# JonasGeiping/breaching

Measured on AMD Instinct MI355X. Metric: attack iters/sec, ResNet-18 ImageNet invertinggradients; PSNR vs ref, higher is better.
Workload: dtype f32

## Files before the change

### breaching_amd/_lib.py

```python

import ctypes
import os
from ctypes import POINTER, Structure, c_char_p, c_double, c_float, c_int, c_int32, c_int64, c_uint32, c_void_p

from . import build as _build

BH_ABI_VERSION = 8
BH_GM_CHUNK = 4096
BH_GM_MAX_PTRS = 448
BH_GM_PARTIAL_STRIDE = 4
BH_GM_MAX_ROWS = 2048
BH_GM_DEFAULT_ROWS = 512
BH_GM_STAT_WORDS = 12
BH_PRIOR_MAX_GRID = 1024
BH_BN_MAX_LAYERS = 448
BH_MT_MAX_PTRS = 112
BH_BN_TILE = 4096
BH_PRIOR_PARTIAL_STRIDE = 2
BH_STATE_WORDS = 16
BH_SCHED_STRIDE = 4
GM_CACHE_AUTO, GM_CACHE_KEEP, GM_CACHE_STREAM, GM_CACHE_STREAM_ALL = 0, 1, 2, 3

GM_KINDS = {
    "cosine-similarity": 0,
# ... 85 lines not shown
    ),
    "bh_bn_plan_size": (
        c_int,
        [c_int32, POINTER(c_int32), POINTER(c_int32), POINTER(c_int32), POINTER(c_int64), POINTER(c_int64), POINTER(c_int64),
         POINTER(c_int64), POINTER(c_int64)],
    ),
    "bh_bn_plan_build": (
        c_int,
        [c_int32, POINTER(c_int32), POINTER(c_int32), POINTER(c_int32), POINTER(c_float), POINTER(BnLayer), POINTER(BnItem),
         c_int64, POINTER(BnItem), c_int64],
    ),
    "bh_bn_bwd_accumulate": (c_int, [c_void_p, c_void_p, c_int32, c_void_p, c_void_p, c_int64, c_void_p, c_void_p, c_void_p, c_void_p]),
    "bh_bn_eval_fwd": (c_int, [c_void_p] * 8 + [c_int32, c_int32, c_int32, c_int32, c_void_p]),
    "bh_bn_eval_slabs": (c_int32, [c_int32, c_int32, c_int32]),
    "bh_bn_eval_bwd": (c_int, [c_void_p] * 14 + [c_int32, c_int32, c_int32, c_void_p]),
    "bh_bn_eval_bwd_bwd": (c_int, [c_void_p] * 14 + [c_int32, c_int32, c_int32, c_void_p]),
    "bh_bn_eval_bwd_bwd2": (c_int, [c_void_p] * 15 + [c_int32, c_int32, c_int32, c_void_p]),
    "bh_ln_fwd": (c_int, [c_void_p] * 6 + [c_int32, c_int32, ctypes.c_float, c_void_p]),
    "bh_ln_bwd": (c_int, [c_void_p] * 8 + [c_int32, c_int32, c_void_p]),
    "bh_ln_bwd_bwd": (c_int, [c_void_p] * 12 + [c_int32, c_int32, c_void_p]),
    "bh_bn_sums": (c_int, [c_int32, POINTER(c_void_p), POINTER(c_int32), c_void_p, c_void_p, c_int64, c_void_p, c_int32, c_int32, c_void_p]),
    "bh_bn_finalize": (c_int, [c_int32, c_void_p, c_void_p, c_void_p, c_void_p, c_void_p, c_void_p, c_void_p, c_void_p, c_int32, c_void_p]),
    "bh_bn_bwd": (
        c_int,
        [c_int32, POINTER(c_void_p), POINTER(c_int32), c_void_p, c_void_p, c_int64, c_void_p, c_void_p, c_void_p, c_void_p],
    ),
    "bh_mt_num_groups": (c_int32, [c_int32]),
    "bh_mt_group_bounds": (c_int, [c_int32, POINTER(GmChunk), c_int64, POINTER(c_int32)]),
    "bh_mt_axpy": (
        c_int,
# ... 87 lines not shown
```

### breaching_amd/attacker.py

```python

import copy
import logging
import time
from collections import defaultdict

import numpy as np
import torch

from . import _lib, schedules, streams as trial_streams, trials, workers
from .config import cfg_get as _cfg_get
from .gm import objective_lookup
from .priors import HipNormRegularization, HipTotalVariation, launch_tv_norm, regularizer_lookup
from .victim_layers import (FusedEpilogueError, _ConvFunction, _ConvGradFunction, _EvalAffineBatchNorm2d, _EvalBNFunction,
                            _EvalBNGradFunction, _HipConv2d, _HipLayerNorm, owned_conv_grad_enabled, use_owned_conv_gradient,
                            _launch_eval_bn, _LayerNormFunction, _LayerNormGradFunction, _PendingBatchNorm, _under_functorch,
                            fast_eval_bn_enabled, fast_eval_bn_mode, fast_layer_norm_enabled, fuse_bn_relu_enabled, fuse_bn_relu_policy,
                            use_affine_eval_batchnorm, use_hip_layernorm)

log = logging.getLogger(__name__)

embedding_layer_names = ["encoder.weight", "word_embeddings.weight", "transformer.wte"]

_DEFAULT_SETUP = dict(dtype=torch.float, device=torch.device("cpu"))


class HipOptimizationAttacker:

    def __init__(self, model, loss_fn, cfg_attack, setup=_DEFAULT_SETUP):
        self.cfg = cfg_attack
        self.memory_format = torch.channels_last if cfg_attack.impl.mixed_precision else torch.contiguous_format
        self.setup = dict(device=torch.device(setup["device"]), dtype=getattr(torch, cfg_attack.impl.dtype))
# ... 122 lines not shown
            optimal = self._select_optimal_reconstruction(local_solutions, local_scores, stats, shard)
            timing["select_s"] = time.perf_counter() - t_select
            if pool is not None:
                pool.timing["select_s"] = round(timing["select_s"], 4)
                pool.finish()
        except BaseException:
            if pool is not None:
                pool.abort()
                if pool.closed:
                    self._pool = None
            raise
        timing["total_s"] = time.perf_counter() - t_call
        stats["execution"] = dict(trials=stats.pop("execution_trials"), pool=pool.describe() if pool is not None else None,
                                  fused_epilogue_fallback=getattr(self, "fused_epilogue_fallback", None),
                                  owned_conv_grad=owned_conv_grad_enabled(self.cfg),
                                  pool_fallback=getattr(self, "_pool_fallback", None), world=shard.world,
                                  trial_streams=trial_streams.calibration_report(self.setup["device"]),
                                  timing={k: round(v, 4) for k, v in timing.items()})
        reconstructed_data = self._package(optimal, labels)
        if server_payload[0]["metadata"].modality == "text":
            raw = reconstructed_data["data"]
            reconstructed_data = self._postprocess_text_data(reconstructed_data)
            self._attach_raw_embeddings(reconstructed_data, raw)
        if "ClassAttack" in server_secrets:
            true_num_data = server_secrets["ClassAttack"]["true_num_data"]
            full = torch.zeros([true_num_data, *self.data_shape], **self.setup)
            full[server_secrets["ClassAttack"]["target_indx"]] = optimal if torch.is_tensor(optimal) else optimal[0]
            reconstructed_data["data"] = full
            reconstructed_data["labels"] = server_secrets["ClassAttack"]["all_labels"]
        return reconstructed_data, stats
# ... 107 lines not shown
                new_model.train()
                for module in new_model.modules():
                    if hasattr(module, "track_running_stats"):
                        module.reset_parameters()
                        module.track_running_stats = False
                buffers = []
            with torch.no_grad():
                for param, server_state in zip(new_model.parameters(), payload["parameters"]):
                    param.copy_(server_state.to(**self.setup))
                for buffer, server_state in zip(new_model.buffers(), buffers):
                    buffer.copy_(server_state.to(**self.setup))
            if self.cfg.impl.JIT is not None:
                raise NotImplementedError("impl.JIT (torch.jit script/trace of the victim model) is not supported.")
            bn_mode = fast_eval_bn_mode(self.cfg)
            if bn_mode is not None:
                use_affine_eval_batchnorm(new_model, bn_mode, fuse_epilogue=fuse_bn_relu_enabled(self.cfg))
            if fast_layer_norm_enabled(self.cfg):
                use_hip_layernorm(new_model)
            if owned_conv_grad_enabled(self.cfg):
                use_owned_conv_gradient(new_model)
            models.append(new_model)
        return models

    def _cast_shared_data(self, shared_data):
        for data in shared_data:
            data["gradients"] = [g.to(**self.setup) for g in data["gradients"]]
            if data["buffers"] is not None:
                data["buffers"] = [b.to(device=self.setup["device"], dtype=self.setup["dtype"]) for b in data["buffers"]]
        return shared_data

    def _normalize_gradients(self, shared_data, fudge_factor=1e-6):
        for data in shared_data:
            grad_norm = torch.stack([g.pow(2).sum() for g in data["gradients"]]).sum().sqrt()
            torch._foreach_div_(data["gradients"], max(grad_norm, fudge_factor))
        return shared_data
# ... 839 lines not shown
```

### breaching_amd/csrc/affine_kernels.hip

```cpp

#include "bh_common.h"

namespace {

using bh::kBlock;


struct ChannelWalk {
  int c, slab, lane, lanes;
  bool active;
};

__device__ __forceinline__ ChannelWalk channel_of(int C, int S, bool narrow) {
  ChannelWalk w;
  if (narrow) {
    w.c = blockIdx.x * bh::kWavesPerBlock + (threadIdx.x >> 6);
    w.slab = 0;
    w.lane = threadIdx.x & (bh::kWave - 1);
    w.lanes = bh::kWave;
  } else {
    w.c = blockIdx.x / S;
    w.slab = blockIdx.x - w.c * S;
    w.lane = threadIdx.x;
    w.lanes = kBlock;
// ... 103 lines not shown
        flush();
      }
    }
    sums[0] += (double)a0;
    sums[1] += (double)a1;
  }
  if (stats == nullptr) return;
  channel_sum<2>(sums, narrow != 0, lds);
  if (w.active && w.lane == 0) {
    double* out = stats + 2 * ((size_t)w.c * S + w.slab);
    out[0] = sums[0];
    out[1] = sums[1];
  }
}

__global__ __launch_bounds__(kBlock) void bn_eval_bwd_kernel(const float* __restrict__ gy, const float* __restrict__ x,
                                                             const float* __restrict__ weight, const float* __restrict__ inv_std,
                                                             const float* __restrict__ mean_inv, float* __restrict__ gx,
                                                             float* __restrict__ gw, float* __restrict__ gb,
                                                             double* __restrict__ part, const float* __restrict__ tap_coef,
                                                             const float* __restrict__ tap_gout, const float* __restrict__ ymask,
                                                             float* __restrict__ gres, const float* __restrict__ add_in, int B, int C,
                                                             int HW, int S, int narrow) {
  __shared__ double lds[bh::kWavesPerBlock * 2];
  const ChannelWalk w = channel_of(C, S, narrow != 0);
  double v[2] = {0.0, 0.0};
  if (w.active) {
    const float s = (weight ? weight[w.c] : 1.f) * inv_std[w.c];
    float ta = 0.f, tb = 0.f;
    if (tap_coef) {
      const float2 ab = reinterpret_cast<const float2*>(tap_coef)[w.c];
      const float g0 = tap_gout ? tap_gout[0] : 1.f;
      ta = g0 * ab.x;
      tb = g0 * ab.y;
    }
    const bool vec = (HW & 3) == 0;
    uint32_t unit, v0, v1;
    slab_range(B, HW, S, w.slab, vec, unit, v0, v1);
    const size_t cstride = (size_t)C * unit, cbase = (size_t)w.c * unit;
    float a0 = 0.f, a1 = 0.f;
    int cnt = 0;
    auto flush = [&]() {
      if (cnt >= 32) {
        v[0] += (double)a0;
        v[1] += (double)a1;
        a0 = a1 = 0.f;
        cnt = 0;
      }
    };
    if (vec) {
      const float4* __restrict__ gy4 = reinterpret_cast<const float4*>(gy);
      const float4* __restrict__ x4 = reinterpret_cast<const float4*>(x);
      const float4* m4 = reinterpret_cast<const float4*>(ymask ? ymask : gy);
      const float4* __restrict__ e4 = reinterpret_cast<const float4*>(add_in);
      float4* __restrict__ gres4 = reinterpret_cast<float4*>(gres);
      float4* __restrict__ gx4 = reinterpret_cast<float4*>(gx);
      const float4 zero = make_float4(0.f, 0.f, 0.f, 0.f);
      const uint32_t step = (uint32_t)w.lanes;
      for (uint32_t u0 = v0 + (uint32_t)w.lane; u0 < v1; u0 += step * kStage) {
        float4 gv[kStage], qv[kStage], mv[kStage], ev[kStage];
        size_t at[kStage];
#pragma unroll
        for (int k = 0; k < kStage; ++k) {
          const uint32_t u = u0 + (uint32_t)k * step;
          at[k] = slab_offset(u < v1 ? u : u0, B, unit, cstride, cbase);
          gv[k] = gy4[at[k]];
          qv[k] = x4[at[k]];
          mv[k] = m4[at[k]];
          ev[k] = zero;
          if (gx && add_in) ev[k] = e4[at[k]];
        }
#pragma unroll
        for (int k = 0; k < kStage; ++k) {
          const uint32_t u = u0 + (uint32_t)k * step;
          if (u < v1) {
            float4 g = gv[k];
            const float4 q = qv[k];
            if (ymask) {
              const float4 m = mv[k];
              g = make_float4(m.x <= 0.f ? 0.f : g.x, m.y <= 0.f ? 0.f : g.y, m.z <= 0.f ? 0.f : g.z, m.w <= 0.f ? 0.f : g.w);
            }
            if (gres) gres4[at[k]] = g;
            if (gx) {
              float4 o = make_float4(g.x * s, g.y * s, g.z * s, g.w * s);
              if (tap_coef) o = make_float4(o.x + fmaf(tb, q.x, ta), o.y + fmaf(tb, q.y, ta), o.z + fmaf(tb, q.z, ta), o.w + fmaf(tb, q.w, ta));
              if (add_in) {
                const float4 e = ev[k];
                o = make_float4(o.x + e.x, o.y + e.y, o.z + e.z, o.w + e.w);
              }
              gx4[at[k]] = o;
            }
            a0 += (g.x + g.y) + (g.z + g.w);
            a1 = fmaf(g.x, q.x, a1);
            a1 = fmaf(g.y, q.y, a1);
            a1 = fmaf(g.z, q.z, a1);
            a1 = fmaf(g.w, q.w, a1);
            cnt += 4;
            flush();
          }
        }
      }
    } else {
      for (uint32_t u = v0 + (uint32_t)w.lane; u < v1; u += (uint32_t)w.lanes) {
        const size_t at = slab_offset(u, B, unit, cstride, cbase);
        float g = gy[at];
        const float q = x[at];
        if (ymask && ymask[at] <= 0.f) g = 0.f;
        if (gres) gres[at] = g;
        if (gx) gx[at] = (tap_coef ? g * s + fmaf(tb, q, ta) : g * s) + (add_in ? add_in[at] : 0.f);
        a0 += g;
        a1 = fmaf(g, q, a1);
        cnt += 1;
        flush();
      }
    }
    v[0] += (double)a0;
    v[1] += (double)a1;
  }
  channel_sum<2>(v, narrow != 0, lds);
  if (w.active && w.lane == 0) {
    if (S > 1) {
      part[((size_t)w.c * S + w.slab) * 2] = v[0];
      part[((size_t)w.c * S + w.slab) * 2 + 1] = v[1];
// ... 159 lines not shown

int bh_bn_eval_fwd(const float* x, const float* weight, const float* bias, const float* inv_std, const float* mean_inv, float* y,
                   double* stats, const float* residual, int32_t relu, int32_t B, int32_t C, int32_t HW, void* stream) {
  if (!eval_bn_args_ok(x, inv_std, mean_inv, B, C, HW) || y == nullptr) return BH_EINVAL;
  if ((reinterpret_cast<uintptr_t>(stats) & 7u) != 0 || (relu != 0 && relu != 1)) return BH_EINVAL;
  if ((HW & 3) == 0 &&
      ((reinterpret_cast<uintptr_t>(x) | reinterpret_cast<uintptr_t>(y) | reinterpret_cast<uintptr_t>(residual)) & 15u) != 0)
    return BH_EINVAL;
  int S = 1, narrow = 0;
  const int grid = eval_bn_grid(B, C, HW, S, narrow);
  hipLaunchKernelGGL(bn_eval_fwd_kernel, dim3(grid), dim3(kBlock), 0, bh::as_stream(stream), x, weight, bias, inv_std, mean_inv,
                     y, stats, residual, relu, B, C, HW, S, narrow);
  return bh::launch_status();
}

int bh_bn_eval_bwd(const float* gy, const float* x, const float* weight, const float* inv_std, const float* mean_inv, float* gx,
                   float* gw, float* gb, double* workspace, const float* tap_coef, const float* tap_gout, const float* y_mask,
                   float* g_residual, const float* gx_add, int32_t B, int32_t C, int32_t HW, void* stream) {
  if (!eval_bn_args_ok(x, inv_std, mean_inv, B, C, HW) || gy == nullptr) return BH_EINVAL;
  if ((reinterpret_cast<uintptr_t>(tap_coef) & 7u) != 0 || ((tap_coef != nullptr || gx_add != nullptr) && gx == nullptr)) return BH_EINVAL;
  if ((HW & 3) == 0 && ((reinterpret_cast<uintptr_t>(x) | reinterpret_cast<uintptr_t>(gy) | reinterpret_cast<uintptr_t>(gx) |
                         reinterpret_cast<uintptr_t>(y_mask) | reinterpret_cast<uintptr_t>(g_residual) | reinterpret_cast<uintptr_t>(gx_add)) & 15u) != 0)
    return BH_EINVAL;
  int S = 1, narrow = 0;
  const int grid = eval_bn_grid(B, C, HW, S, narrow);
  if (S > 1 && workspace == nullptr) return BH_EINVAL;
  hipStream_t st = bh::as_stream(stream);
  hipLaunchKernelGGL(bn_eval_bwd_kernel, dim3(grid), dim3(kBlock), 0, st, gy, x, weight, inv_std, mean_inv, gx, gw, gb, workspace,
                     tap_coef, tap_gout, y_mask, g_residual, gx_add, B, C, HW, S, narrow);
  if (S > 1 && (gw != nullptr || gb != nullptr))
    hipLaunchKernelGGL(bn_eval_combine_kernel<2>, dim3((C + kBlock - 1) / kBlock), dim3(kBlock), 0, st, workspace, inv_std,
                       mean_inv, gw, gb, C, S);
  return bh::launch_status();
}

int bh_bn_eval_bwd_bwd2(const float* ggx, const float* ggx2, const float* ggw, const float* ggb, const float* gy, const float* x,
                        const float* weight, const float* inv_std, const float* mean_inv, float* d_gy, float* d_x, float* d_w,
                        double* workspace, const float* y_mask, const float* gg_residual, int32_t B, int32_t C, int32_t HW, void* stream) {
  if (!eval_bn_args_ok(x, inv_std, mean_inv, B, C, HW) || gy == nullptr) return BH_EINVAL;
  if (ggx2 != nullptr && ggx == nullptr) return BH_EINVAL;
  if ((HW & 3) == 0 && ((reinterpret_cast<uintptr_t>(x) | reinterpret_cast<uintptr_t>(gy) | reinterpret_cast<uintptr_t>(ggx) |
                         reinterpret_cast<uintptr_t>(ggx2) | reinterpret_cast<uintptr_t>(d_gy) | reinterpret_cast<uintptr_t>(d_x) | reinterpret_cast<uintptr_t>(y_mask) |
                         reinterpret_cast<uintptr_t>(gg_residual)) & 15u) != 0)
    return BH_EINVAL;
  int S = 1, narrow = 0;
  const int grid = eval_bn_grid(B, C, HW, S, narrow);
  if (S > 1 && workspace == nullptr) return BH_EINVAL;
  hipStream_t st = bh::as_stream(stream);
// ... 17 lines not shown
```

### breaching_amd/victim_layers.py

```python

import torch

from . import _lib
from .config import cfg_get as _cfg_get

def _vector_ready(t, hw):
    if not t.is_contiguous():
        t = t.contiguous()
    if hw % 4 == 0 and t.data_ptr() % 16:
        t = t.clone()
    return t


def _under_functorch(x):
    try:
        from torch._C._functorch import is_functorch_wrapped_tensor, peek_interpreter_stack

        return bool(is_functorch_wrapped_tensor(x)) or peek_interpreter_stack() is not None
    except Exception:
        return False


class _EvalBNFunction(torch.autograd.Function):

    @staticmethod
    def forward(ctx, x, weight, bias, inv_std, mean_inv, stats=None, tap=None, residual=None, relu=False):
        lib = _lib.load()
        B, C = x.shape[0], x.shape[1]
        hw = x[0, 0].numel()
        xk = _vector_ready(x.detach(), hw)
        rk = None if residual is None else _vector_ready(residual.detach().to(torch.float32), hw)
        y = torch.empty_like(xk)
        with torch.cuda.device(x.device):
            _lib.check(lib.bh_bn_eval_fwd(_lib.ptr(xk), _lib.ptr(weight), _lib.ptr(bias), _lib.ptr(inv_std), _lib.ptr(mean_inv),
                                          _lib.ptr(y), _lib.ptr(stats), _lib.ptr(rk), int(bool(relu)), B, C, hw,
                                          _lib.current_stream_handle(x.device)), "bh_bn_eval_fwd")
        xp = x.view_as(x)
        ctx.save_for_backward(xp, weight, inv_std, mean_inv, *([y] if relu else []))
        ctx.has_bias, ctx.relu, ctx.has_residual = bias is not None, bool(relu), residual is not None
        ctx.tap = None if tap is None else (tap.record, tap.layer)
        ctx.set_materialize_grads(False)
        return (y, xp) if tap is None else (y, xp, x.new_empty(()))

    @staticmethod
    def backward(ctx, gy, g_xp=None, g_token=None):
        xp, weight, inv_std, mean_inv, *rest = ctx.saved_tensors
        mask = rest[0].detach() if ctx.relu else None
        none = (None,) * 9
        if g_token is None or ctx.tap is None:
            if gy is None:
                return (g_xp,) + none[1:]
            tap = None
        else:
            if torch.is_grad_enabled():
                raise NotImplementedError("The DeepInversion term fused into the BatchNorm backward supports no create_graph "
                                          "pass through it (set BREACH_HIP_BN_FUSED_TAP=0).")
            record, layer = ctx.tap
            _, coef_ptr = record.layer_coefficients(layer)
            if gy is None:
                gy = torch.zeros_like(xp)
            tap = (coef_ptr, g_token.detach().reshape(1).to(torch.float32), record.coef)
        fold = g_xp is not None and not torch.is_grad_enabled()
        gx, gw, gb, gr = _EvalBNGradFunction.apply(gy, xp, weight, inv_std, mean_inv, mask, tap, ctx.has_residual, g_xp if fold else None)
        if g_xp is not None and not fold:
            gx = gx + g_xp
        return gx, (gw if weight is not None else None), (gb if ctx.has_bias else None), None, None, None, None, gr, None


class _EvalBNGradFunction(torch.autograd.Function):

    @staticmethod
    def forward(ctx, gy, x, weight, inv_std, mean_inv, mask=None, tap=None, want_residual=False, gx_add=None):
        lib = _lib.load()
        B, C = x.shape[0], x.shape[1]
        hw = x[0, 0].numel()
        gyk = _vector_ready(gy.detach().to(torch.float32), hw)
        xk = _vector_ready(x.detach(), hw)
        mk = None if mask is None else _vector_ready(mask.detach(), hw)
        ak = None if gx_add is None else _vector_ready(gx_add.detach().to(torch.float32), hw)
        gx = torch.empty_like(xk)
        gr = torch.empty_like(xk) if want_residual else None
        gw = torch.empty(C, dtype=torch.float32, device=x.device)
        gb = torch.empty(C, dtype=torch.float32, device=x.device)
        slabs = lib.bh_bn_eval_slabs(B, C, hw)
        ws = torch.empty(2 * C * slabs, dtype=torch.float64, device=x.device) if slabs > 1 else None
        coef_ptr, gout = (tap[0], _lib.ptr(tap[1])) if tap is not None else (_lib.ptr(None), _lib.ptr(None))
        with torch.cuda.device(x.device):
            _lib.check(lib.bh_bn_eval_bwd(_lib.ptr(gyk), _lib.ptr(xk), _lib.ptr(weight), _lib.ptr(inv_std), _lib.ptr(mean_inv),
                                          _lib.ptr(gx), _lib.ptr(gw), _lib.ptr(gb), _lib.ptr(ws), coef_ptr, gout, _lib.ptr(mk), _lib.ptr(gr),
                                          _lib.ptr(ak), B, C, hw, _lib.current_stream_handle(x.device)), "bh_bn_eval_bwd")
        ctx.save_for_backward(gyk, xk, weight, inv_std, mean_inv, *([mk] if mk is not None else []))
        ctx.set_materialize_grads(False)
        ctx.extra_terms, ctx.masked = (tap is not None or gx_add is not None), mk is not None
        return gx, gw, gb, gr

    @staticmethod
    @torch.autograd.function.once_differentiable
    def backward(ctx, ggx, ggw, ggb, ggr):
        lib = _lib.load()
        gy, x, weight, inv_std, mean_inv, *rest = ctx.saved_tensors
        mask = rest[0] if ctx.masked else None
        none = (None,) * 9
        ggx2 = _take_conv_term(ctx)
        if ggx is None:
            ggx, ggx2 = ggx2, None
        if ggx is None and ggw is None and ggb is None and ggr is None:
            return none
        if ctx.extra_terms:
            raise NotImplementedError("No derivative of the BatchNorm backward with the DeepInversion term / another gradient folded in.")
        B, C = x.shape[0], x.shape[1]
        hw = x[0, 0].numel()
        ggx = None if ggx is None else _vector_ready(ggx.to(torch.float32), hw)
        ggx2 = None if ggx2 is None else _vector_ready(ggx2.to(torch.float32), hw)
        ggr = None if ggr is None else _vector_ready(ggr.to(torch.float32), hw)
        ggw = None if ggw is None else ggw.to(torch.float32).contiguous()
        ggb = None if ggb is None else ggb.to(torch.float32).contiguous()
        d_gy = torch.empty_like(x) if ctx.needs_input_grad[0] else None
        d_x = torch.empty_like(x) if (ctx.needs_input_grad[1] and ggw is not None) else None
        d_w = torch.empty(C, dtype=torch.float32, device=x.device) if (weight is not None and ctx.needs_input_grad[2] and ggx is not None) else None
        if d_gy is None and d_x is None and d_w is None:
            return none
        slabs = lib.bh_bn_eval_slabs(B, C, hw)
        ws = torch.empty(C * slabs, dtype=torch.float64, device=x.device) if slabs > 1 else None
        with torch.cuda.device(x.device):
            _lib.check(lib.bh_bn_eval_bwd_bwd2(_lib.ptr(ggx), _lib.ptr(ggx2), _lib.ptr(ggw), _lib.ptr(ggb), _lib.ptr(gy), _lib.ptr(x),
                                               _lib.ptr(weight), _lib.ptr(inv_std), _lib.ptr(mean_inv), _lib.ptr(d_gy), _lib.ptr(d_x),
                                               _lib.ptr(d_w), _lib.ptr(ws), _lib.ptr(mask), _lib.ptr(ggr), B, C, hw,
                                               _lib.current_stream_handle(x.device)), "bh_bn_eval_bwd_bwd2")
        return d_gy, d_x, d_w, None, None, None, None, None, None


def _take_conv_term(node):
    entry = getattr(node, "_conv_term", None)
    if entry is None:
        return None
    node._conv_term = None
    return entry[1] if entry[0] == torch._C._current_graph_task_id() else None


def _engine_wants(edge):
    node = edge[0] if edge is not None else None
    if node is None:
        return False
    try:
        return bool(torch._C._will_engine_execute_node(node))
    except RuntimeError:
        return True


_aten = torch.ops.aten


class _ConvFunction(torch.autograd.Function):

    @staticmethod
    def forward(ctx, x, w, b, stride, padding, dilation, groups):
        ctx.geometry = (list(stride), list(padding), list(dilation), int(groups))
        ctx.bias_sizes = None if b is None else [w.shape[0]]
        ctx.save_for_backward(x, w)
        return _aten.convolution(x, w, b, ctx.geometry[0], ctx.geometry[1], ctx.geometry[2], False, [0] * len(ctx.geometry[0]), groups)

    @staticmethod
    def backward(ctx, gy):
        x, w = ctx.saved_tensors
        none = (None,) * 7
        mask = tuple(bool(ctx.needs_input_grad[i]) and _engine_wants(ctx.next_functions[i]) for i in range(3))
        if not any(mask):
            return none
        producer = gy.grad_fn if gy.output_nr == 0 and getattr(gy.grad_fn, "_forward_cls", None) is _EvalBNGradFunction else None
        gx, gw, gb = _ConvGradFunction.apply(gy, x, w, ctx.geometry, mask, ctx.bias_sizes, producer)
        return (gx, gw, gb) + none[3:]


class _ConvGradFunction(torch.autograd.Function):

    @staticmethod
    def forward(ctx, gy, x, w, geometry, mask, bias_sizes, producer):
        stride, padding, dilation, groups = geometry
        ctx.geometry, ctx.producer = geometry, producer
        ctx.save_for_backward(gy, x, w)
        ctx.set_materialize_grads(False)
        return _aten.convolution_backward(gy, x, w, bias_sizes, stride, padding, dilation, False, [0] * len(stride), groups, list(mask))

    @staticmethod
    @torch.autograd.function.once_differentiable
    def backward(ctx, ggx, ggw, ggb):
        gy, x, w = ctx.saved_tensors
        stride, padding, dilation, groups = ctx.geometry
        zeros = [0] * len(stride)
        want = [bool(ctx.needs_input_grad[i]) and _engine_wants(ctx.next_functions[i]) for i in range(3)]
        d_gy = d_x = d_w = None
        if want[0]:
            t1 = None if ggx is None else _aten.convolution(ggx, w, None, stride, padding, dilation, False, zeros, groups)
            t2 = None if ggw is None else _aten.convolution(x, ggw, None, stride, padding, dilation, False, zeros, groups)
            if t1 is not None and t2 is not None:
                d_gy = t1 if ggb is None and _leave_on_producer(ctx, t2) else t1 + t2
            else:
                d_gy = t1 if t2 is None else t2
            if ggb is not None:
                bias = ggb.reshape(1, -1, *([1] * (gy.dim() - 2)))
                d_gy = bias.expand_as(gy) if d_gy is None else d_gy + bias
        if want[1] and ggw is not None:
            d_x = _aten.convolution_backward(gy, x, ggw, None, stride, padding, dilation, False, zeros, groups, [True, False, False])[0]
        if want[2] and ggx is not None:
            d_w = _aten.convolution_backward(gy, ggx, w, None, stride, padding, dilation, False, zeros, groups, [False, True, False])[1]
        return d_gy, d_x, d_w, None, None, None, None


def _leave_on_producer(ctx, term):
    producer = ctx.producer
    if producer is None or ctx.next_functions[0] != (producer, 0):
        return False
    try:
        if not torch._C._will_engine_execute_node(producer):
            return False
    except RuntimeError:
        return False
    task = torch._C._current_graph_task_id()
    entry = getattr(producer, "_conv_term", None)
    if entry is not None and entry[0] == task:
        term = entry[1] + term
    producer._conv_term = (task, term)
    return True


class _HipConv2d(torch.nn.Conv2d):

    def forward(self, x):
        if isinstance(x, _PendingBatchNorm):
            x = x.value()
        if (self.padding_mode != "zeros" or isinstance(self.padding, str) or x.dim() != 4 or not x.is_floating_point()
                or x.dtype != self.weight.dtype or torch.is_autocast_enabled(x.device.type) or _under_functorch(x)):
            return super().forward(x)
        return _ConvFunction.apply(x, self.weight, self.bias, self.stride, self.padding, self.dilation, self.groups)


def use_owned_conv_gradient(model):
    for module in model.modules():
        if type(module) is torch.nn.Conv2d:
            module.__class__ = _HipConv2d
    return model


def owned_conv_grad_enabled(cfg):
    import os

    env = os.environ.get("BREACH_HIP_CONV_GRAD")
    if env is not None:
        return env.strip().lower() not in ("0", "false", "off", "no")
    flag = _cfg_get(cfg.impl, "owned_conv_grad", True)
    return True if flag is None else bool(flag)


def _launch_eval_bn(module, x, sink, tap, residual, relu):
    inv_std, mean_inv = module._frozen_statistics()
    out = _EvalBNFunction.apply(x, module.weight, module.bias, inv_std, mean_inv, sink, tap, residual, relu)
    if tap is not None:
        tap.token = out[2]
    return out[0]


_RELU_OUT_OF_PLACE = (torch.relu, torch.nn.functional.relu, torch.Tensor.relu)
_RELU_IN_PLACE = (torch.relu_, torch.Tensor.relu_, torch.nn.functional.relu_)
_ADD_OUT_OF_PLACE = (torch.add, torch.Tensor.add, torch.Tensor.__add__, torch.Tensor.__radd__)
_ADD_IN_PLACE = (torch.Tensor.add_, torch.Tensor.__iadd__)


class FusedEpilogueError(RuntimeError):
    """The deferred BatchNorm launch (`_PendingBatchNorm`) met a consumer it cannot serve.  With cfg.impl.fuse_bn_relu = "auto" (the
    default) the attacker catches it on the model copy it happened on, switches the epilogue fusion off there and repeats the
    evaluation; "required" lets it through."""
# ... 99 lines not shown
        flag = flag.strip().lower()
        if flag in ("required", "require", "strict"):
            return "required"
        return "off" if flag in ("0", "false", "off", "no") else "auto"
    return "auto" if bool(flag) else "off"


def fuse_bn_relu_enabled(cfg=None):
    return fuse_bn_relu_policy(cfg) != "off"


class _EvalAffineBatchNorm2d(torch.nn.BatchNorm2d):

    eval_mode = "hip"
    fuse_epilogue = True

    def _runs_on_hip(self, x):
        if not (not self.training and self.running_mean is not None and self.running_var is not None and x.dim() == 4
                and self.eval_mode == "hip" and x.is_cuda and x.dtype == torch.float32 and x.numel() > 0):
            return False
        if x.shape[0] * x.shape[2] * x.shape[3] >= 2 ** 31 or x.numel() >= 2 ** 40:
            return False
        return not _under_functorch(x)

    def accepts_stats_sink(self, x):
        return self._runs_on_hip(x)

    def forward(self, x):
        if isinstance(x, _PendingBatchNorm):
            x = x.value()
# ... 19 lines not shown
        if self.bias is not None:
            shift = shift + self.bias
        return torch.addcmul(shift.view(1, -1, 1, 1), x, scale.view(1, -1, 1, 1))

    def _frozen_statistics(self):
        key = (self.running_mean._version, self.running_var._version, self.running_var.data_ptr(), self.running_var.device)
        cached = getattr(self, "_frozen", None)
        if cached is None or cached[0] != key:
            with torch.no_grad():
                inv_std = torch.rsqrt(self.running_var + self.eps).to(torch.float32).contiguous()
                cached = (key, inv_std, (self.running_mean * inv_std).to(torch.float32).contiguous())
            self._frozen = cached
        return cached[1], cached[2]


def use_affine_eval_batchnorm(model, mode="hip", fuse_epilogue=True):
    for module in model.modules():
        if type(module) is torch.nn.BatchNorm2d:
            module.__class__ = _EvalAffineBatchNorm2d
        if type(module) is _EvalAffineBatchNorm2d:
            module.eval_mode = mode
            module.fuse_epilogue = bool(fuse_epilogue)
    return model


def fast_eval_bn_mode(cfg):
    import os

    flag = os.environ.get("BREACH_HIP_FAST_BN")
    if flag is None:
        flag = _cfg_get(cfg.impl, "fast_eval_bn", True)
    if flag is None or flag is True:
        return "hip"
    if flag is False:
        return None
    flag = str(flag).strip().lower()
    if flag in ("0", "false", "off", "no", "stock"):
# ... 105 lines not shown
```

### include/breach_hip.h

```cpp
#ifndef BREACH_HIP_H
#define BREACH_HIP_H

#include <stdint.h>

#ifdef __cplusplus
extern "C" {
#endif

#define BH_ABI_VERSION 8
#define BH_EINVAL (-1)


#ifndef BH_GM_CHUNK
#define BH_GM_CHUNK 4096
#endif
#define BH_GM_MAX_PTRS 448
#define BH_GM_PARTIAL_STRIDE 4
#define BH_GM_MAX_ROWS 2048
#define BH_GM_DEFAULT_ROWS 512

typedef struct bh_gm_chunk {
  int64_t flat_off;
  int64_t tensor_off;
  int32_t tensor;
// ... 107 lines not shown

int bh_bn_bwd(int32_t n_layers, const void* const* x_ptrs, const int32_t* hw_host, const bh_bn_layer* layers_dev,
              const bh_bn_item* bwd_items_dev, int64_t n_bwd_items, const float* coef_dev, const float* gout_dev,
              float* grad_flat, void* stream);

int bh_bn_bwd_accumulate(const float* x, const float* gin, int32_t hw, const bh_bn_layer* layers_dev,
                         const bh_bn_item* layer_bwd_items_dev, int64_t n_items, const float* coef_dev, const float* gout_dev,
                         float* out, void* stream);

int bh_bn_eval_fwd(const float* x, const float* weight, const float* bias, const float* inv_std, const float* mean_inv, float* y,
                   double* stats, const float* residual, int32_t relu, int32_t B, int32_t C, int32_t HW, void* stream);
int32_t bh_bn_eval_slabs(int32_t B, int32_t C, int32_t HW);
int bh_bn_eval_bwd(const float* gy, const float* x, const float* weight, const float* inv_std, const float* mean_inv, float* gx,
                   float* gw, float* gb, double* workspace, const float* tap_coef, const float* tap_gout, const float* y_mask,
                   float* g_residual, const float* gx_add, int32_t B, int32_t C, int32_t HW, void* stream);
int bh_bn_eval_bwd_bwd(const float* ggx, const float* ggw, const float* ggb, const float* gy, const float* x, const float* weight,
                       const float* inv_std, const float* mean_inv, float* d_gy, float* d_x, float* d_w, double* workspace,
                       const float* y_mask, const float* gg_residual, int32_t B, int32_t C, int32_t HW, void* stream);
int bh_bn_eval_bwd_bwd2(const float* ggx, const float* ggx2, const float* ggw, const float* ggb, const float* gy, const float* x,
                        const float* weight, const float* inv_std, const float* mean_inv, float* d_gy, float* d_x, float* d_w,
                        double* workspace, const float* y_mask, const float* gg_residual, int32_t B, int32_t C, int32_t HW, void* stream);

int bh_ln_fwd(const float* x, const float* gamma, const float* beta, float* y, float* mean, float* rstd, int32_t R, int32_t D,
              float eps, void* stream);
int bh_ln_bwd(const float* gy, const float* x, const float* gamma, const float* mean, const float* rstd, float* gx, float* ggamma,
              float* gbeta, int32_t R, int32_t D, void* stream);
int bh_ln_bwd_bwd(const float* u, const float* s, const float* t, const float* gy, const float* x, const float* gamma,
                  const float* mean, const float* rstd, float* d_gy, float* d_x, float* d_gamma, float* row_scalars, int32_t R,
                  int32_t D, void* stream);

// ... 101 lines not shown
```

Measured before the change: 341.4.

## Fold autograd gradient accumulation into eval-BN backward kernel operands

Adds a side channel that lets conv and BN backward nodes deposit their input-gradient terms directly on the downstream eval-BN node, instead of returning them for the autograd engine to sum. The BN backward kernel gains a second gradient input and a residual-add input, so the branch sums for residual connections in ResNet are fused into the kernel's loads and stores. It also skips the weight/bias gradient buffers when the engine does not need them. This relies on private autograd internals (graph task id, will_engine_execute_node) and grows the ABI, which is brittle across PyTorch versions and for graph shapes the code does not anticipate.

```diff
diff --git a/breaching_amd/_lib.py b/breaching_amd/_lib.py
--- a/breaching_amd/_lib.py
+++ b/breaching_amd/_lib.py
@@ -5,7 +5,7 @@
 
 from . import build as _build
 
-BH_ABI_VERSION = 8
+BH_ABI_VERSION = 9
 BH_GM_CHUNK = 4096
 BH_GM_MAX_PTRS = 448
 BH_GM_PARTIAL_STRIDE = 4
@@ -123,6 +123,7 @@
     "bh_bn_eval_fwd": (c_int, [c_void_p] * 8 + [c_int32, c_int32, c_int32, c_int32, c_void_p]),
     "bh_bn_eval_slabs": (c_int32, [c_int32, c_int32, c_int32]),
     "bh_bn_eval_bwd": (c_int, [c_void_p] * 14 + [c_int32, c_int32, c_int32, c_void_p]),
+    "bh_bn_eval_bwd2": (c_int, [c_void_p] * 16 + [c_int32, c_int32, c_int32, c_void_p]),
     "bh_bn_eval_bwd_bwd": (c_int, [c_void_p] * 14 + [c_int32, c_int32, c_int32, c_void_p]),
     "bh_bn_eval_bwd_bwd2": (c_int, [c_void_p] * 15 + [c_int32, c_int32, c_int32, c_void_p]),
     "bh_ln_fwd": (c_int, [c_void_p] * 6 + [c_int32, c_int32, ctypes.c_float, c_void_p]),
diff --git a/breaching_amd/attacker.py b/breaching_amd/attacker.py
--- a/breaching_amd/attacker.py
+++ b/breaching_amd/attacker.py
@@ -14,7 +14,8 @@
 from .victim_layers import (FusedEpilogueError, _ConvFunction, _ConvGradFunction, _EvalAffineBatchNorm2d, _EvalBNFunction,
                             _EvalBNGradFunction, _HipConv2d, _HipLayerNorm, owned_conv_grad_enabled, use_owned_conv_gradient,
                             _launch_eval_bn, _LayerNormFunction, _LayerNormGradFunction, _PendingBatchNorm, _under_functorch,
-                            fast_eval_bn_enabled, fast_eval_bn_mode, fast_layer_norm_enabled, fuse_bn_relu_enabled, fuse_bn_relu_policy,
+                            fast_eval_bn_enabled, fast_eval_bn_mode, fast_layer_norm_enabled, fold_grad_accumulation_enabled,
+                            fuse_bn_relu_enabled, fuse_bn_relu_policy,
                             use_affine_eval_batchnorm, use_hip_layernorm)
 
 log = logging.getLogger(__name__)
@@ -167,6 +168,7 @@
         stats["execution"] = dict(trials=stats.pop("execution_trials"), pool=pool.describe() if pool is not None else None,
                                   fused_epilogue_fallback=getattr(self, "fused_epilogue_fallback", None),
                                   owned_conv_grad=owned_conv_grad_enabled(self.cfg),
+                                  fold_grad_accumulation=fold_grad_accumulation_enabled(self.cfg),
                                   pool_fallback=getattr(self, "_pool_fallback", None), world=shard.world,
                                   trial_streams=trial_streams.calibration_report(self.setup["device"]),
                                   timing={k: round(v, 4) for k, v in timing.items()})
@@ -304,11 +306,12 @@
                 raise NotImplementedError("impl.JIT (torch.jit script/trace of the victim model) is not supported.")
             bn_mode = fast_eval_bn_mode(self.cfg)
             if bn_mode is not None:
-                use_affine_eval_batchnorm(new_model, bn_mode, fuse_epilogue=fuse_bn_relu_enabled(self.cfg))
+                use_affine_eval_batchnorm(new_model, bn_mode, fuse_epilogue=fuse_bn_relu_enabled(self.cfg),
+                                          fold_accum=fold_grad_accumulation_enabled(self.cfg))
             if fast_layer_norm_enabled(self.cfg):
                 use_hip_layernorm(new_model)
             if owned_conv_grad_enabled(self.cfg):
-                use_owned_conv_gradient(new_model)
+                use_owned_conv_gradient(new_model, fold_accum=fold_grad_accumulation_enabled(self.cfg))
             models.append(new_model)
         return models
 
diff --git a/breaching_amd/csrc/affine_kernels.hip b/breaching_amd/csrc/affine_kernels.hip
--- a/breaching_amd/csrc/affine_kernels.hip
+++ b/breaching_amd/csrc/affine_kernels.hip
@@ -141,14 +141,16 @@
   }
 }
 
-__global__ __launch_bounds__(kBlock) void bn_eval_bwd_kernel(const float* __restrict__ gy, const float* __restrict__ x,
+__global__ __launch_bounds__(kBlock) void bn_eval_bwd_kernel(const float* __restrict__ gy, const float* __restrict__ gy2,
+                                                             const float* __restrict__ x,
                                                              const float* __restrict__ weight, const float* __restrict__ inv_std,
                                                              const float* __restrict__ mean_inv, float* __restrict__ gx,
                                                              float* __restrict__ gw, float* __restrict__ gb,
                                                              double* __restrict__ part, const float* __restrict__ tap_coef,
                                                              const float* __restrict__ tap_gout, const float* __restrict__ ymask,
-                                                             float* __restrict__ gres, const float* __restrict__ add_in, int B, int C,
-                                                             int HW, int S, int narrow) {
+                                                             float* __restrict__ gres, const float* __restrict__ add_in,
+                                                             const float* __restrict__ res_add, int B, int C, int HW, int S,
+                                                             int narrow) {
   __shared__ double lds[bh::kWavesPerBlock * 2];
   const ChannelWalk w = channel_of(C, S, narrow != 0);
   double v[2] = {0.0, 0.0};
@@ -177,15 +179,17 @@
     };
     if (vec) {
       const float4* __restrict__ gy4 = reinterpret_cast<const float4*>(gy);
+      const float4* __restrict__ gy24 = reinterpret_cast<const float4*>(gy2);
       const float4* __restrict__ x4 = reinterpret_cast<const float4*>(x);
       const float4* m4 = reinterpret_cast<const float4*>(ymask ? ymask : gy);
       const float4* __restrict__ e4 = reinterpret_cast<const float4*>(add_in);
+      const float4* __restrict__ ra4 = reinterpret_cast<const float4*>(res_add);
       float4* __restrict__ gres4 = reinterpret_cast<float4*>(gres);
       float4* __restrict__ gx4 = reinterpret_cast<float4*>(gx);
       const float4 zero = make_float4(0.f, 0.f, 0.f, 0.f);
       const uint32_t step = (uint32_t)w.lanes;
       for (uint32_t u0 = v0 + (uint32_t)w.lane; u0 < v1; u0 += step * kStage) {
-        float4 gv[kStage], qv[kStage], mv[kStage], ev[kStage];
+        float4 gv[kStage], g2v[kStage], qv[kStage], mv[kStage], ev[kStage];
         size_t at[kStage];
 #pragma unroll
         for (int k = 0; k < kStage; ++k) {
@@ -194,7 +198,8 @@
           gv[k] = gy4[at[k]];
           qv[k] = x4[at[k]];
           mv[k] = m4[at[k]];
-          ev[k] = zero;
+          g2v[k] = ev[k] = zero;
+          if (gy2) g2v[k] = gy24[at[k]];
           if (gx && add_in) ev[k] = e4[at[k]];
         }
 #pragma unroll
@@ -202,12 +207,20 @@
           const uint32_t u = u0 + (uint32_t)k * step;
           if (u < v1) {
             float4 g = gv[k];
+            if (gy2) g = make_float4(g.x + g2v[k].x, g.y + g2v[k].y, g.z + g2v[k].z, g.w + g2v[k].w);
             const float4 q = qv[k];
             if (ymask) {
               const float4 m = mv[k];
               g = make_float4(m.x <= 0.f ? 0.f : g.x, m.y <= 0.f ? 0.f : g.y, m.z <= 0.f ? 0.f : g.z, m.w <= 0.f ? 0.f : g.w);
             }
-            if (gres) gres4[at[k]] = g;
+            if (gres) {
+              float4 o = g;
+              if (res_add) {
+                const float4 e = ra4[at[k]];
+                o = make_float4(e.x + g.x, e.y + g.y, e.z + g.z, e.w + g.w);
+              }
+              gres4[at[k]] = o;
+            }
             if (gx) {
               float4 o = make_float4(g.x * s, g.y * s, g.z * s, g.w * s);
               if (tap_coef) o = make_float4(o.x + fmaf(tb, q.x, ta), o.y + fmaf(tb, q.y, ta), o.z + fmaf(tb, q.z, ta), o.w + fmaf(tb, q.w, ta));
@@ -231,9 +244,10 @@
       for (uint32_t u = v0 + (uint32_t)w.lane; u < v1; u += (uint32_t)w.lanes) {
         const size_t at = slab_offset(u, B, unit, cstride, cbase);
         float g = gy[at];
+        if (gy2) g = g + gy2[at];
         const float q = x[at];
         if (ymask && ymask[at] <= 0.f) g = 0.f;
-        if (gres) gres[at] = g;
+        if (gres) gres[at] = res_add ? res_add[at] + g : g;
         if (gx) gx[at] = (tap_coef ? g * s + fmaf(tb, q, ta) : g * s) + (add_in ? add_in[at] : 0.f);
         a0 += g;
         a1 = fmaf(g, q, a1);
@@ -423,24 +437,34 @@
   return bh::launch_status();
 }
 
-int bh_bn_eval_bwd(const float* gy, const float* x, const float* weight, const float* inv_std, const float* mean_inv, float* gx,
-                   float* gw, float* gb, double* workspace, const float* tap_coef, const float* tap_gout, const float* y_mask,
-                   float* g_residual, const float* gx_add, int32_t B, int32_t C, int32_t HW, void* stream) {
+int bh_bn_eval_bwd2(const float* gy, const float* gy2, const float* x, const float* weight, const float* inv_std,
+                    const float* mean_inv, float* gx, float* gw, float* gb, double* workspace, const float* tap_coef,
+                    const float* tap_gout, const float* y_mask, float* g_residual, const float* gx_add, const float* g_residual_add,
+                    int32_t B, int32_t C, int32_t HW, void* stream) {
   if (!eval_bn_args_ok(x, inv_std, mean_inv, B, C, HW) || gy == nullptr) return BH_EINVAL;
+  if (g_residual_add != nullptr && g_residual == nullptr) return BH_EINVAL;
   if ((reinterpret_cast<uintptr_t>(tap_coef) & 7u) != 0 || ((tap_coef != nullptr || gx_add != nullptr) && gx == nullptr)) return BH_EINVAL;
   if ((HW & 3) == 0 && ((reinterpret_cast<uintptr_t>(x) | reinterpret_cast<uintptr_t>(gy) | reinterpret_cast<uintptr_t>(gx) |
-                         reinterpret_cast<uintptr_t>(y_mask) | reinterpret_cast<uintptr_t>(g_residual) | reinterpret_cast<uintptr_t>(gx_add)) & 15u) != 0)
+                         reinterpret_cast<uintptr_t>(y_mask) | reinterpret_cast<uintptr_t>(g_residual) | reinterpret_cast<uintptr_t>(gx_add) |
+                         reinterpret_cast<uintptr_t>(gy2) | reinterpret_cast<uintptr_t>(g_residual_add)) & 15u) != 0)
     return BH_EINVAL;
   int S = 1, narrow = 0;
   const int grid = eval_bn_grid(B, C, HW, S, narrow);
   if (S > 1 && workspace == nullptr) return BH_EINVAL;
   hipStream_t st = bh::as_stream(stream);
-  hipLaunchKernelGGL(bn_eval_bwd_kernel, dim3(grid), dim3(kBlock), 0, st, gy, x, weight, inv_std, mean_inv, gx, gw, gb, workspace,
-                     tap_coef, tap_gout, y_mask, g_residual, gx_add, B, C, HW, S, narrow);
+  hipLaunchKernelGGL(bn_eval_bwd_kernel, dim3(grid), dim3(kBlock), 0, st, gy, gy2, x, weight, inv_std, mean_inv, gx, gw, gb,
+                     workspace, tap_coef, tap_gout, y_mask, g_residual, gx_add, g_residual_add, B, C, HW, S, narrow);
   if (S > 1 && (gw != nullptr || gb != nullptr))
     hipLaunchKernelGGL(bn_eval_combine_kernel<2>, dim3((C + kBlock - 1) / kBlock), dim3(kBlock), 0, st, workspace, inv_std,
                        mean_inv, gw, gb, C, S);
   return bh::launch_status();
+}
+
+int bh_bn_eval_bwd(const float* gy, const float* x, const float* weight, const float* inv_std, const float* mean_inv, float* gx,
+                   float* gw, float* gb, double* workspace, const float* tap_coef, const float* tap_gout, const float* y_mask,
+                   float* g_residual, const float* gx_add, int32_t B, int32_t C, int32_t HW, void* stream) {
+  return bh_bn_eval_bwd2(gy, nullptr, x, weight, inv_std, mean_inv, gx, gw, gb, workspace, tap_coef, tap_gout, y_mask, g_residual,
+                         gx_add, nullptr, B, C, HW, stream);
 }
 
 int bh_bn_eval_bwd_bwd2(const float* ggx, const float* ggx2, const float* ggw, const float* ggb, const float* gy, const float* x,
diff --git a/breaching_amd/victim_layers.py b/breaching_amd/victim_layers.py
--- a/breaching_amd/victim_layers.py
+++ b/breaching_amd/victim_layers.py
@@ -24,7 +24,7 @@
 class _EvalBNFunction(torch.autograd.Function):
 
     @staticmethod
-    def forward(ctx, x, weight, bias, inv_std, mean_inv, stats=None, tap=None, residual=None, relu=False):
+    def forward(ctx, x, weight, bias, inv_std, mean_inv, stats=None, tap=None, residual=None, relu=False, fold_accum=None):
         lib = _lib.load()
         B, C = x.shape[0], x.shape[1]
         hw = x[0, 0].numel()
@@ -38,6 +38,9 @@
         xp = x.view_as(x)
         ctx.save_for_backward(xp, weight, inv_std, mean_inv, *([y] if relu else []))
         ctx.has_bias, ctx.relu, ctx.has_residual = bias is not None, bool(relu), residual is not None
+        ctx.fold_accum = fold_grad_accumulation_enabled() if fold_accum is None else bool(fold_accum)
+        edges = [i for i, a in enumerate((x, weight, bias, inv_std, mean_inv, stats, tap, residual)) if torch.is_tensor(a)]
+        ctx.edge_of = {name: edges.index(i) for name, i in (("weight", 1), ("bias", 2), ("residual", 7)) if i in edges}
         ctx.tap = None if tap is None else (tap.record, tap.layer)
         ctx.set_materialize_grads(False)
         return (y, xp) if tap is None else (y, xp, x.new_empty(()))
@@ -46,7 +49,15 @@
     def backward(ctx, gy, g_xp=None, g_token=None):
         xp, weight, inv_std, mean_inv, *rest = ctx.saved_tensors
         mask = rest[0].detach() if ctx.relu else None
-        none = (None,) * 9
+        none = (None,) * 10
+        terms = _take_terms(ctx)
+        if gy is not None:
+            terms.insert(0, gy)
+        gy, gy2 = (terms[0] if terms else None), None
+        if len(terms) > 1:
+            for term in terms[1:-1]:
+                gy = gy + term
+            gy2 = terms[-1]
         if g_token is None or ctx.tap is None:
             if gy is None:
                 return (g_xp,) + none[1:]
@@ -61,16 +72,28 @@
                 gy = torch.zeros_like(xp)
             tap = (coef_ptr, g_token.detach().reshape(1).to(torch.float32), record.coef)
         fold = g_xp is not None and not torch.is_grad_enabled()
-        gx, gw, gb, gr = _EvalBNGradFunction.apply(gy, xp, weight, inv_std, mean_inv, mask, tap, ctx.has_residual, g_xp if fold else None)
+        want_wb, residual_add, target = (True, True), None, None
+        if ctx.fold_accum:
+            want_wb = tuple(name in ctx.edge_of and _engine_wants(ctx.next_functions[ctx.edge_of[name]]) for name in ("weight", "bias"))
+            if ctx.has_residual and _accepts_terms(ctx.next_functions[ctx.edge_of["residual"]]):
+                target = ctx.next_functions[ctx.edge_of["residual"]][0]
+                if not torch.is_grad_enabled() and len(_peek_terms(target)) == 1:
+                    residual_add = _take_terms(target)[0]
+        gx, gw, gb, gr = _EvalBNGradFunction.apply(gy, xp, weight, inv_std, mean_inv, mask, tap, ctx.has_residual, g_xp if fold else None,
+                                                   gy2, residual_add, want_wb)
         if g_xp is not None and not fold:
             gx = gx + g_xp
-        return gx, (gw if weight is not None else None), (gb if ctx.has_bias else None), None, None, None, None, gr, None
+        if target is not None:
+            _deposit_term(ctx.next_functions[ctx.edge_of["residual"]], gr)
+            gr = None
+        return gx, (gw if weight is not None else None), (gb if ctx.has_bias else None), None, None, None, None, gr, None, None
 
 
 class _EvalBNGradFunction(torch.autograd.Function):
 
     @staticmethod
-    def forward(ctx, gy, x, weight, inv_std, mean_inv, mask=None, tap=None, want_residual=False, gx_add=None):
+    def forward(ctx, gy, x, weight, inv_std, mean_inv, mask=None, tap=None, want_residual=False, gx_add=None, gy2=None,
+                residual_add=None, want_wb=(True, True)):
         lib = _lib.load()
         B, C = x.shape[0], x.shape[1]
         hw = x[0, 0].numel()
@@ -78,21 +101,26 @@
         xk = _vector_ready(x.detach(), hw)
         mk = None if mask is None else _vector_ready(mask.detach(), hw)
         ak = None if gx_add is None else _vector_ready(gx_add.detach().to(torch.float32), hw)
+        g2k = None if gy2 is None else _vector_ready(gy2.detach().to(torch.float32), hw)
+        rak = None if residual_add is None else _vector_ready(residual_add.detach().to(torch.float32), hw)
+        keep_sum = g2k is not None and any(ctx.needs_input_grad)
         gx = torch.empty_like(xk)
-        gr = torch.empty_like(xk) if want_residual else None
-        gw = torch.empty(C, dtype=torch.float32, device=x.device)
-        gb = torch.empty(C, dtype=torch.float32, device=x.device)
+        gr = torch.empty_like(xk) if (want_residual or keep_sum) else None
+        gw = torch.empty(C, dtype=torch.float32, device=x.device) if want_wb[0] else None
+        gb = torch.empty(C, dtype=torch.float32, device=x.device) if want_wb[1] else None
         slabs = lib.bh_bn_eval_slabs(B, C, hw)
         ws = torch.empty(2 * C * slabs, dtype=torch.float64, device=x.device) if slabs > 1 else None
         coef_ptr, gout = (tap[0], _lib.ptr(tap[1])) if tap is not None else (_lib.ptr(None), _lib.ptr(None))
         with torch.cuda.device(x.device):
-            _lib.check(lib.bh_bn_eval_bwd(_lib.ptr(gyk), _lib.ptr(xk), _lib.ptr(weight), _lib.ptr(inv_std), _lib.ptr(mean_inv),
-                                          _lib.ptr(gx), _lib.ptr(gw), _lib.ptr(gb), _lib.ptr(ws), coef_ptr, gout, _lib.ptr(mk), _lib.ptr(gr),
-                                          _lib.ptr(ak), B, C, hw, _lib.current_stream_handle(x.device)), "bh_bn_eval_bwd")
-        ctx.save_for_backward(gyk, xk, weight, inv_std, mean_inv, *([mk] if mk is not None else []))
+            _lib.check(lib.bh_bn_eval_bwd2(_lib.ptr(gyk), _lib.ptr(g2k), _lib.ptr(xk), _lib.ptr(weight), _lib.ptr(inv_std),
+                                           _lib.ptr(mean_inv), _lib.ptr(gx), _lib.ptr(gw), _lib.ptr(gb), _lib.ptr(ws), coef_ptr, gout,
+                                           _lib.ptr(mk), _lib.ptr(gr), _lib.ptr(ak), _lib.ptr(rak), B, C, hw,
+                                           _lib.current_stream_handle(x.device)), "bh_bn_eval_bwd2")
+        ctx.save_for_backward(gr if keep_sum else gyk, xk, weight, inv_std, mean_inv, *([mk] if mk is not None else []))
         ctx.set_materialize_grads(False)
-        ctx.extra_terms, ctx.masked = (tap is not None or gx_add is not None), mk is not None
-        return gx, gw, gb, gr
+        ctx.extra_terms, ctx.masked = (tap is not None or gx_add is not None or rak is not None), mk is not None
+        ctx.two_terms = g2k is not None
+        return gx, gw, gb, (gr if want_residual else None)
 
     @staticmethod
     @torch.autograd.function.once_differentiable
@@ -100,7 +128,7 @@
         lib = _lib.load()
         gy, x, weight, inv_std, mean_inv, *rest = ctx.saved_tensors
         mask = rest[0] if ctx.masked else None
-        none = (None,) * 9
+        none = (None,) * 12
         ggx2 = _take_conv_term(ctx)
         if ggx is None:
             ggx, ggx2 = ggx2, None
@@ -115,7 +143,7 @@
         ggr = None if ggr is None else _vector_ready(ggr.to(torch.float32), hw)
         ggw = None if ggw is None else ggw.to(torch.float32).contiguous()
         ggb = None if ggb is None else ggb.to(torch.float32).contiguous()
-        d_gy = torch.empty_like(x) if ctx.needs_input_grad[0] else None
+        d_gy = torch.empty_like(x) if (ctx.needs_input_grad[0] or (ctx.two_terms and ctx.needs_input_grad[9])) else None
         d_x = torch.empty_like(x) if (ctx.needs_input_grad[1] and ggw is not None) else None
         d_w = torch.empty(C, dtype=torch.float32, device=x.device) if (weight is not None and ctx.needs_input_grad[2] and ggx is not None) else None
         if d_gy is None and d_x is None and d_w is None:
@@ -127,7 +155,7 @@
                                                _lib.ptr(weight), _lib.ptr(inv_std), _lib.ptr(mean_inv), _lib.ptr(d_gy), _lib.ptr(d_x),
                                                _lib.ptr(d_w), _lib.ptr(ws), _lib.ptr(mask), _lib.ptr(ggr), B, C, hw,
                                                _lib.current_stream_handle(x.device)), "bh_bn_eval_bwd_bwd2")
-        return d_gy, d_x, d_w, None, None, None, None, None, None
+        return d_gy, d_x, d_w, None, None, None, None, None, None, (d_gy if ctx.two_terms else None), None, None
 
 
 def _take_conv_term(node):
@@ -136,6 +164,49 @@
         return None
     node._conv_term = None
     return entry[1] if entry[0] == torch._C._current_graph_task_id() else None
+
+
+def _accepts_terms(edge):
+    node, input_nr = edge if edge is not None else (None, 0)
+    if node is None or input_nr != 0 or getattr(node, "_forward_cls", None) is not _EvalBNFunction:
+        return False
+    try:
+        return bool(torch._C._will_engine_execute_node(node))
+    except RuntimeError:
+        return False
+
+
+def _peek_terms(node):
+    entry = getattr(node, "_accum_terms", None)
+    return entry[1] if entry is not None and entry[0] == torch._C._current_graph_task_id() else []
+
+
+def _take_terms(node):
+    terms = _peek_terms(node)
+    if getattr(node, "_accum_terms", None) is not None:
+        node._accum_terms = None
+    return list(terms)
+
+
+def _deposit_term(edge, term):
+    if term is None or not _accepts_terms(edge):
+        return False
+    node, task = edge[0], torch._C._current_graph_task_id()
+    entry = getattr(node, "_accum_terms", None)
+    if entry is None or entry[0] != task:
+        entry = node._accum_terms = (task, [])
+    entry[1].append(term)
+    return True
+
+
+def fold_grad_accumulation_enabled(cfg=None):
+    import os
+
+    env = os.environ.get("BREACH_HIP_FOLD_ACCUM")
+    if env is not None:
+        return env.strip().lower() not in ("0", "false", "off", "no")
+    flag = _cfg_get(cfg.impl, "fold_grad_accumulation", True) if cfg is not None else True
+    return True if flag is None else bool(flag)
 
 
 def _engine_wants(edge):
@@ -154,8 +225,9 @@
 class _ConvFunction(torch.autograd.Function):
 
     @staticmethod
-    def forward(ctx, x, w, b, stride, padding, dilation, groups):
+    def forward(ctx, x, w, b, stride, padding, dilation, groups, fold_accum=None):
         ctx.geometry = (list(stride), list(padding), list(dilation), int(groups))
+        ctx.fold_accum = fold_grad_accumulation_enabled() if fold_accum is None else bool(fold_accum)
         ctx.bias_sizes = None if b is None else [w.shape[0]]
         ctx.save_for_backward(x, w)
         return _aten.convolution(x, w, b, ctx.geometry[0], ctx.geometry[1], ctx.geometry[2], False, [0] * len(ctx.geometry[0]), groups)
@@ -163,21 +235,23 @@
     @staticmethod
     def backward(ctx, gy):
         x, w = ctx.saved_tensors
-        none = (None,) * 7
+        none = (None,) * 8
         mask = tuple(bool(ctx.needs_input_grad[i]) and _engine_wants(ctx.next_functions[i]) for i in range(3))
         if not any(mask):
             return none
         producer = gy.grad_fn if gy.output_nr == 0 and getattr(gy.grad_fn, "_forward_cls", None) is _EvalBNGradFunction else None
-        gx, gw, gb = _ConvGradFunction.apply(gy, x, w, ctx.geometry, mask, ctx.bias_sizes, producer)
+        gx, gw, gb = _ConvGradFunction.apply(gy, x, w, ctx.geometry, mask, ctx.bias_sizes, producer, ctx.fold_accum)
+        if ctx.fold_accum and _deposit_term(ctx.next_functions[0], gx):
+            gx = None
         return (gx, gw, gb) + none[3:]
 
 
 class _ConvGradFunction(torch.autograd.Function):
 
     @staticmethod
-    def forward(ctx, gy, x, w, geometry, mask, bias_sizes, producer):
+    def forward(ctx, gy, x, w, geometry, mask, bias_sizes, producer, fold_accum=False):
         stride, padding, dilation, groups = geometry
-        ctx.geometry, ctx.producer = geometry, producer
+        ctx.geometry, ctx.producer, ctx.fold_accum = geometry, producer, bool(fold_accum)
         ctx.save_for_backward(gy, x, w)
         ctx.set_materialize_grads(False)
         return _aten.convolution_backward(gy, x, w, bias_sizes, stride, padding, dilation, False, [0] * len(stride), groups, list(mask))
@@ -204,7 +278,9 @@
             d_x = _aten.convolution_backward(gy, x, ggw, None, stride, padding, dilation, False, zeros, groups, [True, False, False])[0]
         if want[2] and ggx is not None:
             d_w = _aten.convolution_backward(gy, ggx, w, None, stride, padding, dilation, False, zeros, groups, [False, True, False])[1]
-        return d_gy, d_x, d_w, None, None, None, None
+        if ctx.fold_accum and _deposit_term(ctx.next_functions[1], d_x):
+            d_x = None
+        return d_gy, d_x, d_w, None, None, None, None, None
 
 
 def _leave_on_producer(ctx, term):
@@ -226,19 +302,23 @@
 
 class _HipConv2d(torch.nn.Conv2d):
 
+    fold_accum = None
+
     def forward(self, x):
         if isinstance(x, _PendingBatchNorm):
             x = x.value()
         if (self.padding_mode != "zeros" or isinstance(self.padding, str) or x.dim() != 4 or not x.is_floating_point()
                 or x.dtype != self.weight.dtype or torch.is_autocast_enabled(x.device.type) or _under_functorch(x)):
             return super().forward(x)
-        return _ConvFunction.apply(x, self.weight, self.bias, self.stride, self.padding, self.dilation, self.groups)
-
-
-def use_owned_conv_gradient(model):
+        return _ConvFunction.apply(x, self.weight, self.bias, self.stride, self.padding, self.dilation, self.groups, self.fold_accum)
+
+
+def use_owned_conv_gradient(model, fold_accum=None):
     for module in model.modules():
         if type(module) is torch.nn.Conv2d:
             module.__class__ = _HipConv2d
+        if type(module) is _HipConv2d and fold_accum is not None:
+            module.fold_accum = bool(fold_accum)
     return model
 
 
@@ -254,7 +334,7 @@
 
 def _launch_eval_bn(module, x, sink, tap, residual, relu):
     inv_std, mean_inv = module._frozen_statistics()
-    out = _EvalBNFunction.apply(x, module.weight, module.bias, inv_std, mean_inv, sink, tap, residual, relu)
+    out = _EvalBNFunction.apply(x, module.weight, module.bias, inv_std, mean_inv, sink, tap, residual, relu, module.fold_accum)
     if tap is not None:
         tap.token = out[2]
     return out[0]
@@ -384,6 +464,7 @@
 
     eval_mode = "hip"
     fuse_epilogue = True
+    fold_accum = None
 
     def _runs_on_hip(self, x):
         if not (not self.training and self.running_mean is not None and self.running_var is not None and x.dim() == 4
@@ -433,13 +514,15 @@
         return cached[1], cached[2]
 
 
-def use_affine_eval_batchnorm(model, mode="hip", fuse_epilogue=True):
+def use_affine_eval_batchnorm(model, mode="hip", fuse_epilogue=True, fold_accum=None):
     for module in model.modules():
         if type(module) is torch.nn.BatchNorm2d:
             module.__class__ = _EvalAffineBatchNorm2d
         if type(module) is _EvalAffineBatchNorm2d:
             module.eval_mode = mode
             module.fuse_epilogue = bool(fuse_epilogue)
+            if fold_accum is not None:
+                module.fold_accum = bool(fold_accum)
     return model
 
 
diff --git a/include/breach_hip.h b/include/breach_hip.h
--- a/include/breach_hip.h
+++ b/include/breach_hip.h
@@ -7,7 +7,7 @@
 extern "C" {
 #endif
 
-#define BH_ABI_VERSION 8
+#define BH_ABI_VERSION 9
 #define BH_EINVAL (-1)
 
 
@@ -145,6 +145,10 @@
 int bh_bn_eval_bwd(const float* gy, const float* x, const float* weight, const float* inv_std, const float* mean_inv, float* gx,
                    float* gw, float* gb, double* workspace, const float* tap_coef, const float* tap_gout, const float* y_mask,
                    float* g_residual, const float* gx_add, int32_t B, int32_t C, int32_t HW, void* stream);
+int bh_bn_eval_bwd2(const float* gy, const float* gy2, const float* x, const float* weight, const float* inv_std,
+                    const float* mean_inv, float* gx, float* gw, float* gb, double* workspace, const float* tap_coef,
+                    const float* tap_gout, const float* y_mask, float* g_residual, const float* gx_add, const float* g_residual_add,
+                    int32_t B, int32_t C, int32_t HW, void* stream);
 int bh_bn_eval_bwd_bwd(const float* ggx, const float* ggw, const float* ggb, const float* gy, const float* x, const float* weight,
                        const float* inv_std, const float* mean_inv, float* d_gy, float* d_x, float* d_w, double* workspace,
                        const float* y_mask, const float* gg_residual, int32_t B, int32_t C, int32_t HW, void* stream);
```

New measurement: 352.7 (median of 6 runs). 1.03x the previous value.
